# vovach777/llcomp

Measured on AMD Instinct MI355X. Metric: encode+decode MPix/s on 4K RGB8, bit-exact, higher is better.
Workload: dtype int32

## Files before the change

llcomp_amd/__init__.py:

```python
import ctypes as C
from collections import namedtuple

import numpy as np

from . import _lib
from ._lib import Info, Opts, OutputFormat

EXT = ".llcomp"
FORMAT_LEGACY, FORMAT_SLICED = 0, 1
(OK, BAD_MAGIC, BAD_EXPONENT, TRUNCATED, BAD_ARGS, OUT_OF_RANGE, OUTPUT_OVERFLOW, HIP_ERROR, NO_DEVICE, NOMEM, BUSY, DEVICE_FAILED) = range(12)
JOB_ENCODE, JOB_DECODE, JOB_DECODE_REGIONS, JOB_DECODE_RESIZED_REGIONS = 0, 1, 2, 3
DTYPE_U8, DTYPE_F32, DTYPE_F16, DTYPE_BF16 = 0, 1, 2, 3
LAYOUT_HWC, LAYOUT_CHW = 0, 1

RawImage = namedtuple("RawImage", "pixels width height channels")


class LlcompError(RuntimeError):
    def __init__(self, status, detail=None):
        self.status = int(status)
        msg = _lib.load().llcomp_mi_strerror(int(status)).decode()
        self.device_error = last_device_error() if self.status == DEVICE_FAILED else None
        super().__init__(msg if not detail else f"{msg} ({detail})")

# ... 626 lines not shown
    lens = (C.c_size_t * n)(*[len(b) for b in bands])
    out, m = _lib.u8p(), C.c_size_t()
    _check(L.llcomp_mi_merge_bands(ptrs, lens, n, C.byref(out), C.byref(m)))
    try:
        return C.string_at(out, m.value)
    finally:
        L.llcomp_mi_free(out)


def split_band(data, tile_row0, tile_row1):
    L = _lib.load()
    data = bytes(data)
    buf = (C.c_uint8 * max(1, len(data))).from_buffer_copy(data or b"\0")
    out, m = _lib.u8p(), C.c_size_t()
    _check(L.llcomp_mi_split_band(C.cast(buf, _lib.u8p), len(data), tile_row0, tile_row1, C.byref(out), C.byref(m)))
    try:
        return C.string_at(out, m.value)
    finally:
        L.llcomp_mi_free(out)


class Codec:

    def __init__(self, frames, w, h, c, tile_w=0, tile_h=0, planar=False, device=-1, small_model=False):
        self._L = _lib.load()
        self._h = C.c_void_p()
        _check(self._L.llcomp_mi_codec_create_ex(C.byref(self._h), device, frames, w, h, c, tile_w, tile_h, int(bool(planar)), 1 if small_model else 0))
        self.frames, self.w, self.h, self.c = frames, w, h, c
        self.n_slices = self._L.llcomp_mi_codec_slices(self._h)
        self.max_payload_bytes = self._L.llcomp_mi_codec_max_payload_bytes(self._h)
        self.workspace_bytes = self._L.llcomp_mi_codec_workspace_bytes(self._h)
        fam = self._L.llcomp_mi_codec_kernel_family(self._h)
        self.family = {"rows": bool(fam & 1), "lds_table": bool(fam & 2), "snapshot": bool(fam & 16), "bank_cache": bool(fam & 32),
                       "lane_shift": (fam >> 8) & 0xFF, "slices_per_wave": (fam >> 16) & 0xFF}

    def close(self):
        if self._h:
            self._L.llcomp_mi_codec_destroy(self._h)
            self._h = None

    __del__ = close

    def encode(self, d_px, d_payload, payload_cap, d_slice_len, d_total, d_status, stream=0):
        _check(self._L.llcomp_mi_codec_encode(self._h, d_px, d_payload, payload_cap, d_slice_len, d_total, d_status, stream))

    def decode(self, d_payload, payload_bytes, d_slice_len, d_px, d_status, stream=0):
        _check(self._L.llcomp_mi_codec_decode(self._h, d_payload, payload_bytes, d_slice_len, d_px, d_status, stream))

    def decode_region(self, d_payload, payload_bytes, d_slice_len, x, y, rw, rh, d_px, d_status, stream=0):
        _check(self._L.llcomp_mi_codec_decode_region(self._h, d_payload, payload_bytes, d_slice_len, x, y, rw, rh, d_px, d_status, stream))

    def encode_region(self, d_payload, payload_bytes, d_slice_len, x, y, rw, rh, d_rect, d_sub_payload, sub_payload_cap, d_sub_len, d_sub_total,
                      d_status, stream=0):
        _check(self._L.llcomp_mi_codec_encode_region(self._h, d_payload or None, payload_bytes, d_slice_len or None, x, y, rw, rh, d_rect,
                                                     d_sub_payload, sub_payload_cap, d_sub_len, d_sub_total, d_status, stream))

    def update_region(self, d_payload, payload_bytes, d_slice_len, x, y, rw, rh, d_rect, d_payload_out, payload_cap, d_slice_len_out, d_total,
                      d_status, stream=0):
        _check(self._L.llcomp_mi_codec_update_region(self._h, d_payload or None, payload_bytes, d_slice_len or None, x, y, rw, rh, d_rect,
                                                     d_payload_out, payload_cap, d_slice_len_out, d_total, d_status, stream))

    def region_family(self, x, y, rw, rh):
        fam = self._L.llcomp_mi_codec_region_family(self._h, x, y, rw, rh)
        if not fam:
            return None
        return {"rows": bool(fam & 1), "lds_table": bool(fam & 2), "snapshot": bool(fam & 16), "bank_cache": bool(fam & 32),
                "lane_shift": (fam >> 8) & 0xFF, "slices_per_wave": (fam >> 16) & 0xFF}
# ... 79 lines not shown
```

llcomp_amd/csrc/codec.hip:

```cpp
#include <hip/hip_runtime.h>

#include <algorithm>
#include <cstdlib>
#include <cstring>
#include <mutex>
#include <new>
#include <vector>

#include "../../include/llcomp_mi.h"
#include "codec_internal.hpp"
#include "container.hpp"
#include "geometry.hpp"
#include "kernels.hpp"
#include "resize.hpp"
#include "snapshot.hpp"
#include "tables.hpp"
#include "update.hpp"

using namespace llcomp_mi;

namespace llcomp_mi {

int status_from_bits(uint32_t bits) {
    if (bits & kStInternal) return LLCOMP_MI_HIP_ERROR;
// ... 741 lines not shown
    DeviceGuard guard(k->device);
    if (!guard.ok) return LLCOMP_MI_HIP_ERROR;
    if (what & LLCOMP_MI_PREPARE_ENCODE) {
        if (snapshot_mode(k->g)) {
            if (int rc = ensure_snapshot_arrays(k, k->g)) return rc;
        }
        if (!snapshot_mode(k->g) || snapshot_chunked(k->g))
            if (int rc = ensure_state_tables(k, k->need_states)) return rc;
    }
    if (what & LLCOMP_MI_PREPARE_DECODE)
        if (int rc = ensure_state_tables(k, k->need_states)) return rc;
    if (what & (LLCOMP_MI_PREPARE_REGION | LLCOMP_MI_PREPARE_REGIONS | LLCOMP_MI_PREPARE_RESIZED | LLCOMP_MI_PREPARE_UPDATE)) {
        if (int rc = ensure_region_arrays(k)) return rc;
        if (region_may_need_states(k))
            if (int rc = ensure_state_tables(k, true)) return rc;
    }
    if (what & LLCOMP_MI_PREPARE_REGIONS)
        if (int rc = ensure_regions_table(k)) return rc;
    if (what & LLCOMP_MI_PREPARE_UPDATE) {
        const uint64_t samples = uint64_t(k->g.frames) * k->g.w * k->g.h * k->g.c;
        if (int rc = ensure_update_arrays(k)) return rc;
        if (int rc = ensure_grown(k, k->d_box, k->box_cap, samples, samples)) return rc;
    }
    if (what & LLCOMP_MI_PREPARE_RESIZED) {
        const uint64_t samples = uint64_t(k->g.frames) * k->g.w * k->g.h * k->g.c;
        if (int rc = ensure_regions_ring(k)) return rc;
        if (int rc = ensure_grown(k, k->d_box, k->box_cap, samples, samples)) return rc;
        if (int rc = ensure_grown(k, k->d_mid, k->mid_cap, samples, samples)) return rc;
    }
    return LLCOMP_MI_OK;
}

uint32_t llcomp_mi_codec_slices(const llcomp_mi_codec* k) { return k ? k->g.n_slices : 0; }
uint32_t llcomp_mi_codec_kernel_family(const llcomp_mi_codec* k) { return k ? (k->g.flags & 0xFFu) | (k->g.lane_shift << 8) | (k->g.lpw << 16) : 0; }
uint64_t llcomp_mi_codec_workspace_bytes(const llcomp_mi_codec* k) { return k ? k->workspace_bytes : 0; }
uint64_t llcomp_mi_codec_allocated_bytes(const llcomp_mi_codec* k) { return k ? k->allocated_bytes : 0; }
uint64_t llcomp_mi_codec_max_payload_bytes(const llcomp_mi_codec* k) {
    return k ? uint64_t(k->g.n_slices) * k->g.slice_cap : 0;
}

int llcomp_mi_codec_model(llcomp_mi_codec* k, const void* d_px, void* d_sym, void* stream) {
    if (!k || !d_px || !d_sym) return LLCOMP_MI_BAD_ARGS;
    DeviceGuard guard(k->device);
    if (!guard.ok) return LLCOMP_MI_HIP_ERROR;
    HIP_TRY(launch_model_fwd(k->g, static_cast<const uint8_t*>(d_px), static_cast<uint32_t*>(d_sym),
                             static_cast<hipStream_t>(stream)));
    return LLCOMP_MI_OK;
}

int llcomp_mi_codec_encode(llcomp_mi_codec* k, const void* d_px, void* d_payload, uint64_t payload_cap, void* d_slice_len,
                           void* d_total, void* d_status, void* stream) {
    if (!k || !d_px || !d_payload || !d_slice_len || !d_total || !d_status) return LLCOMP_MI_BAD_ARGS;
    DeviceGuard guard(k->device);
    if (!guard.ok) return LLCOMP_MI_HIP_ERROR;
    hipStream_t s = static_cast<hipStream_t>(stream);
    DoneGuard done_guard{k, s};
    HIP_TRY(hipMemsetAsync(d_status, 0, 4, s));
    if (int rc = encode_streams(k, k->g, d_px, static_cast<uint32_t*>(d_slice_len), k->d_group_off, static_cast<uint32_t*>(d_status), s)) return rc;
    if (int rc = pack_streams(k, k->g, static_cast<const uint32_t*>(d_slice_len), k->d_group_off, static_cast<uint8_t*>(d_payload), payload_cap,
                              static_cast<uint64_t*>(d_total), static_cast<uint32_t*>(d_status), s))
        return rc;
    ++k->n_encode;
    return LLCOMP_MI_OK;
}

int llcomp_mi_codec_decode(llcomp_mi_codec* k, const void* d_payload, uint64_t payload_bytes, const void* d_slice_len,
                           void* d_px, void* d_status, void* stream) {
    if (!k || !d_payload || !d_slice_len || !d_px || !d_status) return LLCOMP_MI_BAD_ARGS;
    DeviceGuard guard(k->device);
    if (!guard.ok) return LLCOMP_MI_HIP_ERROR;
    hipStream_t s = static_cast<hipStream_t>(stream);
    const Geometry& g = k->g;
    DoneGuard done_guard{k, s};
    HIP_TRY(hipMemsetAsync(d_status, 0, 4, s));
    {
        Timed t(k, s, 7);
        if (int rc = next_state_generation(k, s, k->need_states)) return rc;
    }
    {
        Timed t(k, s, 4);
        HIP_TRY(launch_group_sums(g, static_cast<const uint32_t*>(d_slice_len), k->d_group_off, s));
        HIP_TRY(launch_scan_groups(g, k->d_group_off, k->d_total_tmp, s));
    }
    {
        Timed t(k, s, 4);
        HIP_TRY(launch_stage_streams(g, static_cast<const uint8_t*>(d_payload), payload_bytes,
                                     static_cast<const uint32_t*>(d_slice_len), k->d_group_off, k->d_scratch,
                                     static_cast<uint32_t*>(d_status), s));
    }
    {
        Timed t(k, s, 5);
        const bool cache = use_bank_cache(k, g);
        HIP_TRY(launch_decode_slices(g, k->d_scratch, static_cast<const uint32_t*>(d_slice_len), k->d_states, k->state_generation,
                                     static_cast<int16_t*>(k->d_lane_order), static_cast<uint32_t*>(d_status), k->d_counters, cache, s));
        if (cache) queue_feedback(k, s);
    }
    {
        Timed t(k, s, 6);
        if (model_is_fused(g)) {
            HIP_TRY(launch_model_rows_inv(g, static_cast<const int16_t*>(k->d_lane_order), static_cast<uint8_t*>(d_px), s));
        } else {
            HIP_TRY(launch_from_lane_order_i16(g, static_cast<const int16_t*>(k->d_lane_order),
                                               static_cast<int16_t*>(k->d_sym_or_rec), s));
            HIP_TRY(launch_model_inv(g, static_cast<const int16_t*>(k->d_sym_or_rec), static_cast<uint8_t*>(d_px), s));
        }
    }
    ++k->n_decode;
    return LLCOMP_MI_OK;
}

uint32_t llcomp_mi_codec_region_family(const llcomp_mi_codec* k, uint32_t x, uint32_t y, uint32_t rw, uint32_t rh) {
    RegionBox box;
    Geometry sub;
    if (!k || region_setup(k, x, y, rw, rh, box, sub)) return 0;
    return (sub.flags & 0xFFu) | (sub.lane_shift << 8) | (sub.lpw << 16);
}

int llcomp_mi_codec_decode_region(llcomp_mi_codec* k, const void* d_payload, uint64_t payload_bytes, const void* d_slice_len, uint32_t x,
                                  uint32_t y, uint32_t rw, uint32_t rh, void* d_px, void* d_status, void* stream) {
    if (!k || !d_payload || !d_slice_len || !d_px || !d_status) return LLCOMP_MI_BAD_ARGS;
    RegionBox box;
    Geometry sub;
    if (int rc = region_setup(k, x, y, rw, rh, box, sub)) return rc;
    DeviceGuard guard(k->device);
    if (!guard.ok) return LLCOMP_MI_HIP_ERROR;
    if (int rc = ensure_region_arrays(k)) return rc;
    hipStream_t s = static_cast<hipStream_t>(stream);
    const Geometry& g = k->g;
    DoneGuard done_guard{k, s};
    HIP_TRY(hipMemsetAsync(d_status, 0, 4, s));
    {
        Timed t(k, s, 7);
// ... 431 lines not shown
```

llcomp_amd/csrc/geometry.hpp:

```cpp
#pragma once
#include <algorithm>
#include <cstdint>
#include <cstdlib>

#if defined(__HIPCC__)
#define LLMI_HD __host__ __device__
#else
#define LLMI_HD
#endif

namespace llcomp_mi {

constexpr uint32_t kMaxChannels = 255;

struct Geometry {
    uint32_t frames, w, h, c;
    uint32_t tile_w, tile_h, planar;
    uint32_t ntx, nty;
    uint32_t slices_per_frame;
    uint32_t n_slices;
    uint32_t slice_cap;
    uint32_t nch;
    uint32_t lane_shift;
    uint32_t slice_samples;
    uint32_t lpw;
    uint32_t flags;
};
enum : uint32_t {
    kGeoRows = 1u,
    kGeoLdsTable = 2u,
    kGeoForceReplay = 4u,
    kGeoSmallModel = 8u,
    kGeoSnapshot = 16u,
    kGeoBankCache = 32u,
};
constexpr uint32_t kSnapMaxSamples = 4096;
constexpr uint32_t kSnapMaxChunks = 4;

struct Tuning {
    int lane_shift = -1;
    int lpw = 0;
    bool norows = false;
    bool noldstab = false;
    bool force_replay = false;
    bool nosnap = false;
    bool nocache = false;
    int overlap = 2;
    bool nofeedback = false;
};
inline Tuning tuning_from_env() {
    Tuning t;
    auto num = [](const char* name, long lo, long hi, int dflt) {
        const char* e = std::getenv(name);
        if (!e || !*e) return dflt;
        const long v = std::strtol(e, nullptr, 10);
        return (v >= lo && v <= hi) ? int(v) : dflt;
    };
    auto flag = [](const char* name) { const char* e = std::getenv(name); return e && e[0] == '1'; };
    t.lane_shift = num("LLCOMP_MI_LANE_SHIFT", 0, 6, -1);
    t.lpw = num("LLCOMP_MI_LPW", 1, 64, 0);
    t.norows = flag("LLCOMP_MI_NOROWS");
    t.noldstab = flag("LLCOMP_MI_NOLDSTAB");
    t.force_replay = flag("LLCOMP_MI_FORCE_REPLAY");
    t.nosnap = flag("LLCOMP_MI_NOSNAP");
    t.nocache = flag("LLCOMP_MI_NOCACHE");
    t.nofeedback = flag("LLCOMP_MI_NOFEEDBACK");
    t.overlap = num("LLCOMP_MI_OVERLAP", 0, 2, 2);
    return t;
}

LLMI_HD inline uint32_t snapshot_chunks(const Geometry& g) { return (g.slice_samples + kSnapMaxSamples - 1) / kSnapMaxSamples; }
LLMI_HD inline uint32_t snapshot_cap(const Geometry& g) {
    return g.slice_samples <= kSnapMaxSamples ? (g.slice_samples + 15u) & ~15u : snapshot_chunks(g) * kSnapMaxSamples;
}

constexpr int kBankCacheLog2 = 5;
inline int bank_cache_log2(const Geometry& g) { return (g.flags & kGeoBankCache) ? kBankCacheLog2 : 0; }

LLMI_HD inline uint32_t rows_px_dwords(uint64_t tile_base, uint32_t samples, uint32_t c, uint64_t batch_bytes) {
    if (tile_base + 4 > batch_bytes) return 0;
    const uint64_t k = (batch_bytes - 4 - tile_base) / c + 1;
    return k < samples ? uint32_t(k) : samples;
}
LLMI_HD inline uint32_t rows_px_tail(uint32_t c) { return 1 + (4 + c - 1) / c; }

LLMI_HD inline size_t lane_order_index(const Geometry& g, uint32_t id, uint32_t k) {
    const uint32_t gw = 1u << g.lane_shift;
    return ((size_t(id >> g.lane_shift) * g.slice_samples + k) << g.lane_shift) + (id & (gw - 1));
}

struct SliceRect {
    uint32_t frame, x0, y0, sw, sh, ch;
};

LLMI_HD inline SliceRect slice_rect(const Geometry& g, uint32_t id) {
    SliceRect r;
    r.frame = id / g.slices_per_frame;
    uint32_t s = id - r.frame * g.slices_per_frame;
    uint32_t tile = s;
    r.ch = 0;
    if (g.planar) {
        tile = s / g.c;
        r.ch = s - tile * g.c;
    }
    const uint32_t ty = tile / g.ntx, tx = tile - ty * g.ntx;
    r.x0 = tx * g.tile_w;
    r.y0 = ty * g.tile_h;
    r.sw = g.w - r.x0 < g.tile_w ? g.w - r.x0 : g.tile_w;
    r.sh = g.h - r.y0 < g.tile_h ? g.h - r.y0 : g.tile_h;
    return r;
}

inline uint32_t default_lane_shift(uint32_t n_slices) {
    constexpr uint32_t kMinWaves = 96;
    uint32_t s = 6;
    while (s > 0 && (n_slices >> s) < kMinWaves) --s;
    return s;
// ... 170 lines not shown
```

llcomp_amd/csrc/kernels.hpp:

```cpp
#pragma once
#include <hip/hip_runtime.h>

#include <cstdint>

#include "geometry.hpp"

namespace llcomp_mi {

enum : uint32_t { kStOverflow = 1u, kStBadExponent = 2u, kStTruncated = 4u, kStInternal = 8u  };

enum : uint32_t {
    kCtrDecCachedWaves = 0,
    kCtrDecBypassedWaves = 1,
    kCtrCacheLookups = 2,
    kCtrCacheMisses = 3,
    kCtrCacheWritebacks = 4,
    kCtrDecReplays = 5,
    kCtrEncCarryBacks = 6,
    kCtrGenerationWraps = 7,
    kCtrDecLaunchesCached = 8,
    kCtrDecLaunchesPlainByFeedback = 9,
    kCtrCount = 16,
};

hipError_t launch_model_fwd(const Geometry& g, const uint8_t* d_px, uint32_t* d_sym, hipStream_t stream);
hipError_t launch_model_inv(const Geometry& g, const int16_t* d_rec, uint8_t* d_px, hipStream_t stream);

uint32_t lane_groups(const Geometry& g);
uint32_t slice_capacity_samples(const Geometry& g);
hipError_t launch_to_lane_order_u32(const Geometry& g, const uint32_t* d_img, uint32_t* d_lanes, hipStream_t stream);
hipError_t launch_from_lane_order_i16(const Geometry& g, const int16_t* d_lanes, int16_t* d_img, hipStream_t stream);

bool model_is_fused(const Geometry& g);
bool rows_encoder_reads_pixels(const Geometry& g);
hipError_t launch_model_rows_fwd(const Geometry& g, const uint8_t* d_px, uint16_t* d_lanes, hipStream_t stream);
hipError_t launch_model_rows_inv(const Geometry& g, const int16_t* d_lanes, uint8_t* d_px, hipStream_t stream);

bool rows_mode(const Geometry& g);
bool slices_need_state_tables(const Geometry& g);

hipError_t launch_encode_slices(const Geometry& g, const void* d_sym, uint64_t* d_states, uint32_t generation, uint8_t* d_scratch,
                                uint32_t* d_slice_len, uint64_t* d_group_off, uint32_t* d_status, unsigned long long* d_counters,
                                hipStream_t stream);
uint64_t state_generation_tag(uint32_t generation);
hipError_t launch_encode_segment(const Geometry& g, const void* d_res, uint64_t* d_banks, uint8_t* d_scratch, uint32_t* d_slice_len,
                                 uint32_t* d_status, unsigned long long* d_counters, uint32_t seg_first, uint32_t* d_seg_state,
                                 hipStream_t stream);
bool encoder_writes_group_sums(const Geometry& g);
hipError_t launch_group_sums(const Geometry& g, const uint32_t* d_slice_len, uint64_t* d_group_off, hipStream_t stream);
hipError_t launch_scan_groups(const Geometry& g, uint64_t* d_group_off, uint64_t* d_total, hipStream_t stream);
hipError_t launch_frame_bytes(const Geometry& g, const uint32_t* d_slice_len, uint64_t* d_frame_bytes, hipStream_t stream);
hipError_t launch_pack_payload(const Geometry& g, const uint8_t* d_units, const uint32_t* d_slice_len,
                               const uint64_t* d_group_off, uint8_t* d_payload, uint64_t payload_cap,
                               uint32_t* d_status, hipStream_t stream);
hipError_t launch_stage_streams(const Geometry& g, const uint8_t* d_payload, uint64_t payload_bytes,
                                const uint32_t* d_slice_len, const uint64_t* d_group_off, uint8_t* d_units,
                                uint32_t* d_status, hipStream_t stream);
hipError_t launch_copy_segments(const uint8_t* d_src, uint8_t* d_dst, const uint64_t* d_src_off, const uint64_t* d_dst_off,
                                const uint64_t* d_len, uint32_t n_seg, uint64_t max_len, hipStream_t stream);
hipError_t launch_range_sums(const uint32_t* d_vals, const uint64_t* d_start, const uint64_t* d_count, uint64_t* d_out, uint32_t n,
                             uint32_t cap, hipStream_t stream);
hipError_t launch_decode_slices(const Geometry& g, const uint8_t* d_units, const uint32_t* d_slice_len,
                                uint64_t* d_states, uint32_t generation, int16_t* d_rec, uint32_t* d_status, unsigned long long* d_counters,
                                bool bank_cache, hipStream_t stream);

hipError_t launch_region_index(const Geometry& full, const Geometry& sub, const RegionBox& box, const uint32_t* d_slice_len,
                               const uint64_t* d_group_off, uint32_t* d_sub_len, uint64_t* d_sub_off, hipStream_t stream);
hipError_t launch_stage_region_streams(const Geometry& sub, const uint8_t* d_payload, uint64_t payload_bytes, const uint32_t* d_sub_len,
                                       const uint64_t* d_sub_off, uint8_t* d_units, uint32_t* d_status, hipStream_t stream);
struct Crop {
    uint32_t x0, y0, rw, rh;
};
hipError_t launch_model_inv_crop(const Geometry& sub, const int16_t* d_rec, uint8_t* d_px, const Crop& cr, hipStream_t stream);
hipError_t launch_model_rows_inv_crop(const Geometry& sub, const int16_t* d_lanes, uint8_t* d_px, const Crop& cr, hipStream_t stream);

hipError_t launch_regions_index(const Geometry& full, const Geometry& sub, const RegionsFrame* d_tab, const uint32_t* d_slice_len,
                                const uint64_t* d_group_off, uint32_t* d_sub_len, uint64_t* d_sub_off, hipStream_t stream);
hipError_t launch_model_inv_crops(const Geometry& sub, const int16_t* d_rec, uint8_t* d_px, const RegionsFrame* d_tab, uint32_t rw,
                                  uint32_t rh, hipStream_t stream);
hipError_t launch_model_rows_inv_crops(const Geometry& sub, const int16_t* d_lanes, uint8_t* d_px, const RegionsFrame* d_tab, uint32_t rw,
                                       uint32_t rh, hipStream_t stream);

}
```

llcomp_amd/csrc/model_kernels.hip:

```cpp
#include <algorithm>

#include "device_common.hpp"
#include "kernels.hpp"

namespace llcomp_mi {

namespace {

constexpr int kMW = 256;
constexpr int kMH = 32;

template <int C>
__device__ __forceinline__ void rct_forward(const uint8_t* p, int16_t (&o)[C]) {
    if constexpr (C >= 3) {
        const int g = p[1], cb = int(p[2]) - g, cr = int(p[0]) - g;
        o[0] = int16_t(cr);
        o[1] = int16_t(g + (cb + cr) / 4);
        o[2] = int16_t(cb);
        if constexpr (C == 4) o[3] = p[3];
    } else {
#pragma unroll
        for (int k = 0; k < C; ++k) o[k] = p[k];
    }
}
// ... 813 lines not shown
        uint8_t bytes[4 * C];
#pragma unroll
        for (int i = 0; i < 4; ++i) {
            const int16_t* s = &tile[4 * q4 + i][col0 + tt * C];
            if constexpr (C >= 3) {
                int r = s[0], gg = s[1], bb = s[2];
                gg -= (r + bb) / 4;
                r += gg;
                bb += gg;
                bytes[i * C + 0] = uint8_t(min(max(r, 0), 255));
                bytes[i * C + 1] = uint8_t(min(max(gg, 0), 255));
                bytes[i * C + 2] = uint8_t(min(max(bb, 0), 255));
                if constexpr (C == 4) bytes[i * C + 3] = uint8_t(s[3]);
            } else {
#pragma unroll
                for (int c = 0; c < C; ++c) bytes[i * C + c] = uint8_t(s[c]);
            }
        }
        uint8_t* o = px + tiles[tt].base + size_t(kb) * C;
        const uint32_t npx = sw - kb < 4 ? sw - kb : 4;
        if (npx == 4) {
            uint32_t w[C];
#pragma unroll
            for (int c = 0; c < C; ++c)
                w[c] = uint32_t(bytes[4 * c]) | (uint32_t(bytes[4 * c + 1]) << 8) | (uint32_t(bytes[4 * c + 2]) << 16) |
                       (uint32_t(bytes[4 * c + 3]) << 24);
            __builtin_memcpy(o, w, 4 * C);
        } else {
            for (uint32_t i = 0; i < npx * C; ++i) o[i] = bytes[i];
        }
    }
}

struct RowTileCrop {
    long long base;
    uint32_t klo, khi;
};
template <int C>
__device__ __forceinline__ void load_row_tiles_crop(const Geometry& g, uint32_t first_tile, uint32_t ntiles, const Crop& cr,
                                                    RowTileCrop* tiles) {
    if (threadIdx.x < ntiles) {
        const uint32_t tile = first_tile + threadIdx.x;
        const uint32_t per_frame = g.ntx * g.nty;
        const uint32_t frame = tile / per_frame, rem = tile - frame * per_frame;
        const uint32_t y = rem / g.ntx, tx = rem - y * g.ntx;
        const uint32_t x0 = tx * g.tile_w;
        const uint32_t sw = g.w - x0 < g.tile_w ? g.w - x0 : g.tile_w;
        const uint32_t klo = cr.x0 > x0 ? cr.x0 - x0 : 0u;
        uint32_t khi = cr.x0 + cr.rw > x0 ? min(sw, cr.x0 + cr.rw - x0) : 0u;
        if (y < cr.y0 || y >= cr.y0 + cr.rh || khi <= klo) khi = 0;
        tiles[threadIdx.x].base = ((long long)(size_t(frame) * cr.rh + (y - cr.y0)) * cr.rw + (long long)x0 - (long long)cr.x0) * C;
        tiles[threadIdx.x].klo = klo;
        tiles[threadIdx.x].khi = khi;
    }
}
template <int C>
__global__ __launch_bounds__(256) void k_model_rows_inv_crop(const Geometry g, const int16_t* __restrict__ lanes,
                                                             uint8_t* __restrict__ px, const Crop cr) {
    constexpr int K = 64, TPG = 64 / C + 2;
    __shared__ __attribute__((aligned(4))) int16_t tile[K][64 + C + 1 + ((C + 1) & 1)];
    __shared__ RowTileCrop tiles[TPG];
    const uint32_t chunks = (g.tile_w + K - 1) / K;
    uint32_t group, chunk;
    if (!xcd_chunk_group((g.n_slices + (1u << g.lane_shift) - 1) >> g.lane_shift, chunks, group, chunk)) return;
    const uint32_t k0 = chunk * K;
    const uint32_t gw = 1u << g.lane_shift;
// ... 237 lines not shown
    }
    const uint32_t nbx = (g.w + kMW - 1) / kMW;
    const uint32_t spt = (g.tile_h + kMH - 1) / kMH;
    const uint64_t blocks = uint64_t(nbx) * spt * g.nty * g.frames;
    if (blocks == 0 || blocks > 0x7FFFFFFFull) return hipErrorInvalidValue;
    LLMI_DISPATCH_C(g.c, (k_model_fwd<C><<<dim3(uint32_t(blocks)), dim3(kMW), 0, stream>>>(g, d_px, d_sym)));
    return hipGetLastError();
}

uint32_t lane_groups(const Geometry& g) { return (g.n_slices + (1u << g.lane_shift) - 1) >> g.lane_shift; }
uint32_t slice_capacity_samples(const Geometry& g) { return g.slice_samples; }

hipError_t launch_to_lane_order_u32(const Geometry& g, const uint32_t* d_img, uint32_t* d_lanes, hipStream_t stream) {
    const uint32_t max_n = slice_capacity_samples(g);
    const uint64_t blocks = uint64_t(lane_groups(g)) * ((max_n + 63) / 64);
    if (blocks == 0 || blocks > 0x7FFFFFFFull) return hipErrorInvalidValue;
    k_to_lane_order<uint32_t><<<dim3(uint32_t(blocks)), dim3(256), 0, stream>>>(g, max_n, d_img, d_lanes);
    return hipGetLastError();
}

hipError_t launch_from_lane_order_i16(const Geometry& g, const int16_t* d_lanes, int16_t* d_img, hipStream_t stream) {
    const uint32_t max_n = slice_capacity_samples(g);
    const uint64_t blocks = uint64_t(lane_groups(g)) * ((max_n + 63) / 64);
    if (blocks == 0 || blocks > 0x7FFFFFFFull) return hipErrorInvalidValue;
    k_from_lane_order<int16_t><<<dim3(uint32_t(blocks)), dim3(256), 0, stream>>>(g, max_n, d_lanes, d_img);
    return hipGetLastError();
}

bool model_is_fused(const Geometry& g) { return g.planar && rows_mode(g) && g.c <= 4; }
bool rows_encoder_reads_pixels(const Geometry& g) {
    return model_is_fused(g) && (uint64_t(63 / g.c + 2) * g.tile_w * g.c + 4 < (1ull << 31));
}

hipError_t launch_model_rows_fwd(const Geometry& g, const uint8_t* d_px, uint16_t* d_lanes, hipStream_t stream) {
    const uint64_t blocks = xcd_grid(lane_groups(g), (g.tile_w + 63) / 64);
    if (blocks == 0 || blocks > 0x7FFFFFFFull) return hipErrorInvalidValue;
    LLMI_DISPATCH_C(g.c, (k_model_rows_fwd<C><<<dim3(uint32_t(blocks)), dim3(256), 0, stream>>>(g, d_px, d_lanes)));
    return hipGetLastError();
}

hipError_t launch_model_rows_inv(const Geometry& g, const int16_t* d_lanes, uint8_t* d_px, hipStream_t stream) {
    const uint64_t blocks = xcd_chunk_grid(lane_groups(g), (g.tile_w + 63) / 64);
    if (blocks == 0 || blocks > 0x7FFFFFFFull) return hipErrorInvalidValue;
    LLMI_DISPATCH_C(g.c, (k_model_rows_inv<C><<<dim3(uint32_t(blocks)), dim3(256), 0, stream>>>(g, d_lanes, d_px)));
    return hipGetLastError();
}

hipError_t launch_model_inv(const Geometry& g, const int16_t* d_rec, uint8_t* d_px, hipStream_t stream) {
    const size_t npix = size_t(g.frames) * g.h * g.w;
    if (g.c > 4) {
        k_model_inv_any<<<dim3(uint32_t((npix + 255) / 256)), dim3(256), 0, stream>>>(g, d_rec, d_px, npix);
        return hipGetLastError();
    }
    const uint32_t blocks = uint32_t(std::min<size_t>((npix + 255) / 256, 256 * 16));
    LLMI_DISPATCH_C(g.c, (k_model_inv<C><<<dim3(blocks), dim3(256), 0, stream>>>(g, d_rec, d_px, npix)));
    return hipGetLastError();
}

hipError_t launch_group_sums(const Geometry& g, const uint32_t* d_slice_len, uint64_t* d_group_off, hipStream_t stream) {
    k_group_sums<<<dim3((g.n_slices + kSumThreads - 1) / kSumThreads), dim3(kSumThreads), 0, stream>>>(d_slice_len, g.n_slices, g.lane_shift, d_group_off);
    return hipGetLastError();
}

hipError_t launch_frame_bytes(const Geometry& g, const uint32_t* d_slice_len, uint64_t* d_frame_bytes, hipStream_t stream) {
    k_frame_bytes<<<dim3(g.frames), dim3(256), 0, stream>>>(d_slice_len, g.slices_per_frame, d_frame_bytes);
    return hipGetLastError();
// ... 109 lines not shown
```

llcomp_amd/csrc/slice_kernels.hip:

```cpp
#include <algorithm>

#include "device_common.hpp"
#include "kernels.hpp"

#ifndef LLMI_ASM_ENC
#define LLMI_ASM_ENC 1
#endif
#if LLMI_ASM_ENC
#include "enc_rows_asm.hpp"
#endif
#ifndef LLMI_ASM_DEC
#define LLMI_ASM_DEC 1
#endif
#if LLMI_ASM_DEC
#include "dec_rows_asm.hpp"
#endif

namespace llcomp_mi {

namespace {

#ifdef LLMI_CLOCK_PROBE
constexpr uint32_t kProbeSlots = 1u << 15;
__device__ unsigned long long g_probe[2][kProbeSlots][2];
// ... 859 lines not shown
                                           uint32_t& v) {
    const uint32_t s_low = d.low, s_range = d.range, s_b0 = bank.w[0], s_b1 = bank.w[1], s_b2 = bank.w[2], s_b3 = bank.w[3];
    const unsigned long long s_win = d.win;
    bool ok;
#if LLMI_ASM_DEC
    if constexpr (INLDS) {
        uint32_t left;
        dec_rows_sample_asm(d.low, d.range, d.win, bank.w[0], bank.w[1], bank.w[2], bank.w[3], lds_address(bank.lds), hot, v, left);
        ok = left != 0;
    } else
#endif
    {
        ok = hot ? dec_residual<true, false, INLDS>(d, bank, tab, v) : dec_residual<false, false, INLDS>(d, bank, tab, v);
        hot = 2 * __popcll(__ballot(v != 0)) >= __popcll(__ballot(true));
    }
    const bool ran_dry = (INLDS && LLMI_ASM_DEC != 0) ? false : d.win == 0;
    if (__builtin_expect(!ok || ran_dry || replay_always, 0)) {
        ++d.replays;
        d.low = s_low; d.range = s_range; d.win = s_win;
        bank.w[0] = s_b0; bank.w[1] = s_b1;
        if constexpr (INLDS) {
            bank.w[2] = s_b2; bank.w[3] = s_b3;
            reinterpret_cast<uint32_t*>(bank.lds)[0] = s_b0;
            reinterpret_cast<uint32_t*>(bank.lds)[64] = s_b1;
            reinterpret_cast<uint32_t*>(bank.lds)[128] = s_b2;
            reinterpret_cast<uint32_t*>(bank.lds)[192] = s_b3;
        }
        ok = dec_residual<false, true, INLDS>(d, bank, tab, v);
    }
    return ok;
}

constexpr uint32_t bank_cache_lds_bytes(int log2_entries) { return log2_entries ? (64u * 9u) << log2_entries : 0u; }
template <int NCH, bool ROWS, bool LDSTAB = false, int CACHE = 0>
__global__ __launch_bounds__(64) void k_decode_slices(const Geometry g, const uint32_t lpw_and_flags,
                                                      const uint8_t* __restrict__ units,
                                                      const uint32_t* __restrict__ slice_len,
                                                      uint64_t* __restrict__ states, int16_t* __restrict__ rec,
                                                      uint32_t* status, const uint64_t gpat,
                                                      unsigned long long* __restrict__ counters) {
    __shared__ entry_t tab[128];
    __shared__ uint32_t rowbank[ROWS ? kWideBankWords : 1];
    __shared__ int8_t quant_lut[ROWS ? 1 : 512];
    if constexpr (!ROWS) {
        for (uint32_t i = threadIdx.x; i < 256; i += blockDim.x) {
            quant_lut[i] = int8_t(quant11(int(i) - 128));
            quant_lut[256 + i] = int8_t(quant5(int(i) - 128));
        }
    }
    static_assert(CACHE == 0 || (!ROWS && !LDSTAB && NCH != 0), "the bank cache belongs to the 2-D kernels with tables in HBM");
    static_assert(CACHE == 0 || ((kContexts - 1) >> CACHE) < 0xFF, "bank cache: a context's tag would alias the empty marker");
    __shared__ uint32_t wave_sums[CACHE != 0 ? 2 : 1];
    clear_lds_states<LDSTAB>();
    if constexpr (CACHE != 0) {
        uint32_t* tg = reinterpret_cast<uint32_t*>(dyn_lds + (512u << CACHE));
        for (uint32_t i = threadIdx.x; i < (16u << CACHE); i += blockDim.x) tg[i] = 0xFFFFFFFFu;
        if (threadIdx.x < 2) wave_sums[threadIdx.x] = 0;
    }
    load_table(tab);
    const uint32_t lpw = lpw_and_flags & 0xFF;
    const bool replay_always = (lpw_and_flags >> 8) & 1;
    const bool small_model = (g.flags & kGeoSmallModel) != 0;
    const uint32_t id = blockIdx.x * lpw + threadIdx.x;
    if (threadIdx.x >= lpw || id >= g.n_slices) return;
    const SliceRect r = slice_rect(g, id);
    RangeDec d;
    const uint32_t len = min(slice_len[id], g.slice_cap - 16);
    const uint32_t grp = __builtin_amdgcn_readfirstlane(id >> g.lane_shift);
    const uint32_t lane_in_group = id & ((1u << g.lane_shift) - 1);
    dec_open(d, reinterpret_cast<const uint32_t*>(units) + ((size_t(grp) * (g.slice_cap >> 2)) << g.lane_shift), lane_in_group,
             g.lane_shift, len);

    int16_t* p0 = rec + lane_order_index(g, id, 0);
    const ptrdiff_t GW = ptrdiff_t(1) << g.lane_shift;
    int16_t* const gbase = rec + ((size_t(grp) * g.slice_samples) << g.lane_shift);
    uint32_t hot = 0;
    LLMI_PROBE_START();

    if constexpr (ROWS) {
        for (uint32_t k = 0; k < 12; ++k) rowbank[k * 64 + threadIdx.x] = lds_address(tab) * 0x00010001u;
        int l[NCH], L[NCH];
#pragma unroll
        for (int k = 0; k < NCH; ++k) l[k] = L[k] = 128;
        int held_val = 0;
        uint32_t held_ofs = lane_in_group * 2, next_ofs = held_ofs, step_ofs = 2u << g.lane_shift;
        uint32_t large = small_model ? 0u : ~0u, first = ~0u;
        asm volatile("" : "+v"(large), "+v"(first), "+v"(step_ofs));
        uint8_t* const bank0 = reinterpret_cast<uint8_t*>(rowbank) + threadIdx.x * 4;
        bool bad = false;
        auto pixel = [&]() {
#pragma unroll
            for (int k = 0; k < NCH; ++k) {
                if (window_low(d)) dec_append(d);
                asm volatile("global_store_short %0, %1, %2" : : "v"(held_ofs), "v"(held_val), "s"(gbase) : "memory");
                const int lv = l[k];
                const int dq = (L[k] - lv) & int(large);
                int sg = dq >> 31;
                asm volatile("" : "+v"(sg));
                const uint32_t aq = uint32_t((dq ^ sg) - sg);
                uint32_t o1 = ((aq + 0x7FFFFFFFu) >> 21) & 0x400u, o2 = ((aq + 0x7FFFFFFCu) >> 21) & 0x400u;
                asm volatile("" : "+v"(o1), "+v"(o2));
                uint32_t* bp = reinterpret_cast<uint32_t*>(bank0 + (o1 + o2));
                Bank bank{{bp[0], bp[64], bp[128], bp[192]}, reinterpret_cast<uint8_t*>(bp)};
                uint32_t v = 0;
                if (!dec_sample<true>(d, bank, tab, hot, replay_always, v)) bad = true;
                v = (v ^ uint32_t(sg)) - uint32_t(sg);
                const int val = int(int16_t(uint32_t(lv) + v));
                held_val = val;
                held_ofs = next_ofs;
                next_ofs += step_ofs;
                L[k] = lv ^ ((lv ^ val) & int(first));
                l[k] = val;
            }
            first = 0;
        };
        const uint32_t sw0 = __builtin_amdgcn_readfirstlane(r.sw);
        const uint32_t n_bulk = __builtin_amdgcn_ballot_w64(r.sw != sw0) == 0 ? sw0 : 0;
        uint32_t x = 0;
        for (; x < n_bulk; ++x) pixel();
        for (; x < r.sw; ++x) pixel();
        if (bad) atomicOr(status, kStBadExponent);
        asm volatile("global_store_short %0, %1, %2" : : "v"(held_ofs), "v"(held_val), "s"(gbase) : "memory");
        publish_count(counters, kCtrDecReplays, d.replays);
    } else {
        uint64_t* banks;
        uint32_t bsh;
        if constexpr (LDSTAB) {
            banks = reinterpret_cast<uint64_t*>(dyn_lds);
            bsh = 0;
        } else {
            banks = states + ((size_t(id >> g.lane_shift) * kContexts) << g.lane_shift) + (id & ((1u << g.lane_shift) - 1));
            bsh = g.lane_shift;
        }
        if constexpr (NCH == 0) {
            const uint32_t nch = g.nch;
            const ptrdiff_t px_step = ptrdiff_t(nch) * GW, up = ptrdiff_t(r.sw) * px_step;
            for (uint32_t y = 0; y < r.sh; ++y) {
                for (uint32_t x = 0; x < r.sw; ++x) {
                    for (uint32_t k = 0; k < nch; ++k) {
                        int16_t* q = p0 + ptrdiff_t(y) * up + ptrdiff_t(x) * px_step + ptrdiff_t(k) * GW;
                        if (window_low(d)) dec_append(d);
                        const Hood n = apply_borders(x > 0 ? q[-px_step] : 0, x > 1 ? q[-2 * px_step] : 0, y > 0 ? q[-up] : 0,
                                                     (y > 0 && x > 0) ? q[-up - px_step] : 0, (y > 0 && x + 1 < r.sw) ? q[-up + px_step] : 0,
                                                     y > 1 ? q[-2 * up] : 0, x, y, r.sw);
                        int ctx = context_hash(n, small_model);
                        const bool neg = ctx < 0;
                        if (neg) ctx = -ctx;
                        const uint64_t b64 = bank_fresh<LDSTAB>(banks[size_t(ctx) << bsh], gpat);
                        Bank bank{{uint32_t(b64), uint32_t(b64 >> 32)}, nullptr};
                        uint32_t v;
                        if (!dec_sample<false>(d, bank, tab, hot, replay_always, v)) {
                            atomicOr(status, kStBadExponent);
                            return;
                        }
                                banks[size_t(ctx) << bsh] = bank_tagged<LDSTAB>(uint64_t(bank.w[0]) | (uint64_t(bank.w[1]) << 32), gpat);
// ... 220 lines not shown
    const uint32_t lpw = g.lpw;
    const uint32_t blocks = (g.n_slices + lpw - 1) / lpw;
    uint64_t* const d_group_sum = encoder_writes_group_sums(g) ? d_group_off : nullptr;
    if (rows_encoder_reads_pixels(g)) {
        k_encode_slices<1, true, uint8_t><<<dim3(blocks), dim3(64), LLMI_ASM_ENC ? kRowsEncLdsBytes : 0, stream>>>(
            g, lpw, static_cast<const uint8_t*>(d_sym), d_states, d_scratch, d_slice_len, d_group_sum, d_status, gpat, d_counters);
        return hipGetLastError();
    }
    if (model_is_fused(g)) {
        k_encode_slices<1, true, uint16_t><<<dim3(blocks), dim3(64), LLMI_ASM_ENC ? kRowsEncLdsBytes : 0, stream>>>(
            g, lpw, static_cast<const uint16_t*>(d_sym), d_states, d_scratch, d_slice_len, d_group_sum, d_status, gpat, d_counters);
        return hipGetLastError();
    }
    if (g.flags & kGeoSnapshot) {
        k_encode_slices<0, false, uint32_t, false, true><<<dim3(blocks), dim3(64), LLMI_ASM_ENC ? kRowsEncLdsBytes : 0, stream>>>(
            g, lpw, static_cast<const uint32_t*>(d_sym), d_states, d_scratch, d_slice_len, d_group_sum, d_status, 0, d_counters);
        return hipGetLastError();
    }
    const bool lds = states_in_lds(g);
    LLMI_DISPATCH_SLICE(g.nch, rows_mode(g), lds, {
        auto kernel = k_encode_slices<C, R, uint32_t, T>;
        if (T) {
            const hipError_t e = allow_big_lds(kernel);
            if (e != hipSuccess) return e;
        }
        kernel<<<dim3(blocks), dim3(64), T ? kLdsTableBytes : (R && LLMI_ASM_ENC ? kRowsEncLdsBytes : 0), stream>>>(
            g, lpw, static_cast<const uint32_t*>(d_sym), d_states, d_scratch, d_slice_len, d_group_sum, d_status, gpat, d_counters, 0u, nullptr);
    });
    return hipGetLastError();
}

hipError_t launch_decode_slices(const Geometry& g, const uint8_t* d_units, const uint32_t* d_slice_len,
                                uint64_t* d_states, uint32_t generation, int16_t* d_rec, uint32_t* d_status, unsigned long long* d_counters,
                                bool bank_cache, hipStream_t stream) {
    const uint64_t gpat = slices_need_state_tables(g) ? state_generation_tag(generation) : 0;
    const uint32_t lpw = g.lpw;
    const uint32_t blocks = (g.n_slices + lpw - 1) / lpw;
    const uint32_t arg = lpw | ((g.flags & kGeoForceReplay) ? 0x100u : 0u);
    const bool lds = states_in_lds(g);
    if (bank_cache_log2(g) == kBankCacheLog2 && bank_cache) {
#define LLMI_DECODE_CACHED(NCHV)                                                                                          \
    k_decode_slices<NCHV, false, false, kBankCacheLog2><<<dim3(blocks), dim3(64), bank_cache_lds_bytes(kBankCacheLog2), stream>>>( \
        g, arg, d_units, d_slice_len, d_states, d_rec, d_status, gpat, d_counters)
        switch (g.nch) {
            case 1: LLMI_DECODE_CACHED(1); break;
            case 2: LLMI_DECODE_CACHED(2); break;
            case 3: LLMI_DECODE_CACHED(3); break;
            case 4: LLMI_DECODE_CACHED(4); break;
            default: return hipErrorInvalidValue;
        }
#undef LLMI_DECODE_CACHED
        return hipGetLastError();
    }
    LLMI_DISPATCH_SLICE(g.nch, rows_mode(g), lds, {
        auto kernel = k_decode_slices<C, R, T>;
        if (T) {
            const hipError_t e = allow_big_lds(kernel);
            if (e != hipSuccess) return e;
        }
        kernel<<<dim3(blocks), dim3(64), T ? kLdsTableBytes : 0, stream>>>(g, arg, d_units, d_slice_len, d_states,
                                                                          d_rec, d_status, gpat, d_counters);
    });
    return hipGetLastError();
}

}
```

Baseline: 28890.

## Fuse inverse color model and pixel write into the rows slice decoder

The planar rows decoder now stages decoded samples in LDS and, every eight pixels, applies the inverse RGB transform and writes packed 8-byte pixel words straight to the output image. This removes the separate inverse-model pass over the lane-order buffer. Tiles whose channels span two waves still write int16 samples, and a small straddle kernel converts those afterwards. The price is extra LDS staging and wave barriers inside the serial decode loop, plus partial-store handling at tile edges. An env flag can turn the fused path off.

```diff
diff --git a/llcomp_amd/__init__.py b/llcomp_amd/__init__.py
--- a/llcomp_amd/__init__.py
+++ b/llcomp_amd/__init__.py
@@ -682,7 +682,8 @@
         self.workspace_bytes = self._L.llcomp_mi_codec_workspace_bytes(self._h)
         fam = self._L.llcomp_mi_codec_kernel_family(self._h)
         self.family = {"rows": bool(fam & 1), "lds_table": bool(fam & 2), "snapshot": bool(fam & 16), "bank_cache": bool(fam & 32),
-                       "lane_shift": (fam >> 8) & 0xFF, "slices_per_wave": (fam >> 16) & 0xFF}
+                       "lane_shift": (fam >> 8) & 0xFF, "slices_per_wave": (fam >> 16) & 0xFF,
+                       "px_decoder": bool(fam & (1 << 24))}
 
     def close(self):
         if self._h:
diff --git a/llcomp_amd/csrc/codec.hip b/llcomp_amd/csrc/codec.hip
--- a/llcomp_amd/csrc/codec.hip
+++ b/llcomp_amd/csrc/codec.hip
@@ -797,7 +797,11 @@
 }
 
 uint32_t llcomp_mi_codec_slices(const llcomp_mi_codec* k) { return k ? k->g.n_slices : 0; }
-uint32_t llcomp_mi_codec_kernel_family(const llcomp_mi_codec* k) { return k ? (k->g.flags & 0xFFu) | (k->g.lane_shift << 8) | (k->g.lpw << 16) : 0; }
+uint32_t llcomp_mi_codec_kernel_family(const llcomp_mi_codec* k) {
+    if (!k) return 0;
+    const uint32_t px_decoder = rows_decoder_writes_pixels(k->g) && !k->tune.nofuseddec ? 1u << 24 : 0u;
+    return (k->g.flags & 0xFFu) | (k->g.lane_shift << 8) | (k->g.lpw << 16) | px_decoder;
+}
 uint64_t llcomp_mi_codec_workspace_bytes(const llcomp_mi_codec* k) { return k ? k->workspace_bytes : 0; }
 uint64_t llcomp_mi_codec_allocated_bytes(const llcomp_mi_codec* k) { return k ? k->allocated_bytes : 0; }
 uint64_t llcomp_mi_codec_max_payload_bytes(const llcomp_mi_codec* k) {
@@ -853,16 +857,20 @@
                                      static_cast<const uint32_t*>(d_slice_len), k->d_group_off, k->d_scratch,
                                      static_cast<uint32_t*>(d_status), s));
     }
+    const bool px_decoder = rows_decoder_writes_pixels(g) && !k->tune.nofuseddec;
     {
         Timed t(k, s, 5);
         const bool cache = use_bank_cache(k, g);
         HIP_TRY(launch_decode_slices(g, k->d_scratch, static_cast<const uint32_t*>(d_slice_len), k->d_states, k->state_generation,
-                                     static_cast<int16_t*>(k->d_lane_order), static_cast<uint32_t*>(d_status), k->d_counters, cache, s));
+                                     static_cast<int16_t*>(k->d_lane_order), static_cast<uint32_t*>(d_status), k->d_counters, cache, s,
+                                     px_decoder ? static_cast<uint8_t*>(d_px) : nullptr));
         if (cache) queue_feedback(k, s);
     }
     {
         Timed t(k, s, 6);
-        if (model_is_fused(g)) {
+        if (px_decoder) {
+            HIP_TRY(launch_model_rows_inv_straddle(g, static_cast<const int16_t*>(k->d_lane_order), static_cast<uint8_t*>(d_px), s));
+        } else if (model_is_fused(g)) {
             HIP_TRY(launch_model_rows_inv(g, static_cast<const int16_t*>(k->d_lane_order), static_cast<uint8_t*>(d_px), s));
         } else {
             HIP_TRY(launch_from_lane_order_i16(g, static_cast<const int16_t*>(k->d_lane_order),
diff --git a/llcomp_amd/csrc/geometry.hpp b/llcomp_amd/csrc/geometry.hpp
--- a/llcomp_amd/csrc/geometry.hpp
+++ b/llcomp_amd/csrc/geometry.hpp
@@ -47,6 +47,7 @@
     bool nocache = false;
     int overlap = 2;
     bool nofeedback = false;
+    bool nofuseddec = false;
 };
 inline Tuning tuning_from_env() {
     Tuning t;
@@ -65,6 +66,7 @@
     t.nosnap = flag("LLCOMP_MI_NOSNAP");
     t.nocache = flag("LLCOMP_MI_NOCACHE");
     t.nofeedback = flag("LLCOMP_MI_NOFEEDBACK");
+    t.nofuseddec = flag("LLCOMP_MI_NOFUSEDDEC");
     t.overlap = num("LLCOMP_MI_OVERLAP", 0, 2, 2);
     return t;
 }
@@ -83,6 +85,20 @@
     return k < samples ? uint32_t(k) : samples;
 }
 LLMI_HD inline uint32_t rows_px_tail(uint32_t c) { return 1 + (4 + c - 1) / c; }
+
+constexpr uint32_t kRowsFlush = 8;
+LLMI_HD inline bool rows_tile_in_wave(const Geometry& g, uint32_t id) {
+    const uint32_t first = id - id % g.lpw, end = g.n_slices - first < g.lpw ? g.n_slices : first + g.lpw;
+    const uint32_t t0 = id - id % g.c;
+    return t0 >= first && t0 + g.c <= end;
+}
+LLMI_HD inline uint32_t rows_flush_bytes(uint32_t n, uint32_t c, uint32_t plane) {
+    const uint32_t nb = n * c, lo = 8 * plane;
+    return nb > lo ? (nb - lo < 8 ? nb - lo : 8u) : 0u;
+}
+LLMI_HD constexpr uint32_t rows_flush_pixels(uint32_t c) { return c == 3 ? 4u : 8u / c; }
+LLMI_HD inline uint32_t rows_flush_first_pixel(uint32_t c, uint32_t plane) { return c == 3 ? 2 * plane : 8 * plane / c; }
+LLMI_HD inline size_t rows_straddle_index(const Geometry& g, uint32_t id, uint32_t k) { return size_t(id) * g.slice_samples + k; }
 
 LLMI_HD inline size_t lane_order_index(const Geometry& g, uint32_t id, uint32_t k) {
     const uint32_t gw = 1u << g.lane_shift;
diff --git a/llcomp_amd/csrc/kernels.hpp b/llcomp_amd/csrc/kernels.hpp
--- a/llcomp_amd/csrc/kernels.hpp
+++ b/llcomp_amd/csrc/kernels.hpp
@@ -35,6 +35,9 @@
 bool rows_encoder_reads_pixels(const Geometry& g);
 hipError_t launch_model_rows_fwd(const Geometry& g, const uint8_t* d_px, uint16_t* d_lanes, hipStream_t stream);
 hipError_t launch_model_rows_inv(const Geometry& g, const int16_t* d_lanes, uint8_t* d_px, hipStream_t stream);
+bool rows_decoder_writes_pixels(const Geometry& g);
+bool rows_straddlers(const Geometry& g);
+hipError_t launch_model_rows_inv_straddle(const Geometry& g, const int16_t* d_rec, uint8_t* d_px, hipStream_t stream);
 
 bool rows_mode(const Geometry& g);
 bool slices_need_state_tables(const Geometry& g);
@@ -62,7 +65,7 @@
                              uint32_t cap, hipStream_t stream);
 hipError_t launch_decode_slices(const Geometry& g, const uint8_t* d_units, const uint32_t* d_slice_len,
                                 uint64_t* d_states, uint32_t generation, int16_t* d_rec, uint32_t* d_status, unsigned long long* d_counters,
-                                bool bank_cache, hipStream_t stream);
+                                bool bank_cache, hipStream_t stream, uint8_t* d_px = nullptr);
 
 hipError_t launch_region_index(const Geometry& full, const Geometry& sub, const RegionBox& box, const uint32_t* d_slice_len,
                                const uint64_t* d_group_off, uint32_t* d_sub_len, uint64_t* d_sub_off, hipStream_t stream);
diff --git a/llcomp_amd/csrc/model_kernels.hip b/llcomp_amd/csrc/model_kernels.hip
--- a/llcomp_amd/csrc/model_kernels.hip
+++ b/llcomp_amd/csrc/model_kernels.hip
@@ -869,6 +869,36 @@
     }
 }
 
+constexpr uint32_t kStraddleThreads = 256;
+template <int C>
+__global__ __launch_bounds__(kStraddleThreads) void k_model_rows_inv_straddle(const Geometry g, const int16_t* __restrict__ rec, uint8_t* __restrict__ px) {
+    const uint32_t chunks = (g.tile_w + kStraddleThreads - 1) / kStraddleThreads;
+    const uint32_t m = blockIdx.x / chunks + 1, chunk = blockIdx.x - (m - 1) * chunks;
+    const uint32_t b = m * g.lpw;
+    const uint32_t id0 = b - b % C;
+    if (b == id0 || (b - g.lpw > id0)) return;
+    const SliceRect r = slice_rect(g, id0);
+    const uint32_t k = chunk * kStraddleThreads + threadIdx.x;
+    if (k >= r.sw) return;
+    int s[C];
+#pragma unroll
+    for (int c = 0; c < C; ++c) s[c] = rec[rows_straddle_index(g, id0 + c, k)];
+    uint8_t* o = px + ((size_t(r.frame) * g.h + r.y0) * g.w + r.x0 + k) * C;
+    if constexpr (C >= 3) {
+        int rr = s[0], gg = s[1], bb = s[2];
+        gg -= (rr + bb) / 4;
+        rr += gg;
+        bb += gg;
+        o[0] = uint8_t(min(max(rr, 0), 255));
+        o[1] = uint8_t(min(max(gg, 0), 255));
+        o[2] = uint8_t(min(max(bb, 0), 255));
+        if constexpr (C == 4) o[3] = uint8_t(s[3]);
+    } else {
+#pragma unroll
+        for (int c = 0; c < C; ++c) o[c] = uint8_t(s[c]);
+    }
+}
+
 struct RowTileCrop {
     long long base;
     uint32_t klo, khi;
@@ -1172,6 +1202,18 @@
     return model_is_fused(g) && (uint64_t(63 / g.c + 2) * g.tile_w * g.c + 4 < (1ull << 31));
 }
 
+bool rows_decoder_writes_pixels(const Geometry& g) { return rows_encoder_reads_pixels(g); }
+bool rows_straddlers(const Geometry& g) { return g.lpw % g.c != 0 && g.n_slices > g.lpw; }
+
+hipError_t launch_model_rows_inv_straddle(const Geometry& g, const int16_t* d_rec, uint8_t* d_px, hipStream_t stream) {
+    if (!rows_decoder_writes_pixels(g)) return hipErrorInvalidValue;
+    if (!rows_straddlers(g)) return hipSuccess;
+    const uint64_t blocks = uint64_t((g.n_slices - 1) / g.lpw) * ((g.tile_w + kStraddleThreads - 1) / kStraddleThreads);
+    if (blocks == 0 || blocks > 0x7FFFFFFFull) return hipErrorInvalidValue;
+    LLMI_DISPATCH_C(g.c, (k_model_rows_inv_straddle<C><<<dim3(uint32_t(blocks)), dim3(kStraddleThreads), 0, stream>>>(g, d_rec, d_px)));
+    return hipGetLastError();
+}
+
 hipError_t launch_model_rows_fwd(const Geometry& g, const uint8_t* d_px, uint16_t* d_lanes, hipStream_t stream) {
     const uint64_t blocks = xcd_grid(lane_groups(g), (g.tile_w + 63) / 64);
     if (blocks == 0 || blocks > 0x7FFFFFFFull) return hipErrorInvalidValue;
diff --git a/llcomp_amd/csrc/slice_kernels.hip b/llcomp_amd/csrc/slice_kernels.hip
--- a/llcomp_amd/csrc/slice_kernels.hip
+++ b/llcomp_amd/csrc/slice_kernels.hip
@@ -915,15 +915,66 @@
 }
 
 constexpr uint32_t bank_cache_lds_bytes(int log2_entries) { return log2_entries ? (64u * 9u) << log2_entries : 0u; }
-template <int NCH, bool ROWS, bool LDSTAB = false, int CACHE = 0>
+using lds_i16_ptr = __attribute__((address_space(3))) int16_t*;
+__device__ __forceinline__ void rows_inv_rgb(int& r, int& gg, int& bb) {
+    gg -= (r + bb) / 4;
+    r += gg;
+    bb += gg;
+    r = min(max(r, 0), 255);
+    gg = min(max(gg, 0), 255);
+    bb = min(max(bb, 0), 255);
+}
+__device__ __forceinline__ uint32_t pack4(uint32_t b0, uint32_t b1, uint32_t b2, uint32_t b3) { return b0 | (b1 << 8) | (b2 << 16) | (b3 << 24); }
+template <int C>
+__device__ __forceinline__ void rows_flush_words(lds_i16_ptr q, uint32_t sh, uint32_t& w0, uint32_t& w1) {
+    if constexpr (C == 3) {
+        uint32_t b[12];
+#pragma unroll
+        for (int j = 0; j < 4; ++j) {
+            lds_i16_ptr s = q + j * 64;
+            int r = s[0], gg = s[1], bb = s[2];
+            rows_inv_rgb(r, gg, bb);
+            b[3 * j] = uint32_t(r);
+            b[3 * j + 1] = uint32_t(gg);
+            b[3 * j + 2] = uint32_t(bb);
+        }
+        const uint32_t W0 = pack4(b[0], b[1], b[2], b[3]), W1 = pack4(b[4], b[5], b[6], b[7]), W2 = pack4(b[8], b[9], b[10], b[11]);
+        w0 = uint32_t((W0 | ((unsigned long long)W1 << 32)) >> sh);
+        w1 = uint32_t((W1 | ((unsigned long long)W2 << 32)) >> sh);
+    } else if constexpr (C == 4) {
+        uint32_t w[2];
+#pragma unroll
+        for (int j = 0; j < 2; ++j) {
+            lds_i16_ptr s = q + j * 64;
+            int r = s[0], gg = s[1], bb = s[2];
+            const uint32_t a = uint8_t(s[3]);
+            rows_inv_rgb(r, gg, bb);
+            w[j] = pack4(uint32_t(r), uint32_t(gg), uint32_t(bb), a);
+        }
+        w0 = w[0];
+        w1 = w[1];
+    } else {
+        uint32_t b[8];
+#pragma unroll
+        for (int j = 0; j < 8 / C; ++j)
+#pragma unroll
+            for (int c = 0; c < C; ++c) b[j * C + c] = uint8_t(q[j * 64 + c]);
+        w0 = pack4(b[0], b[1], b[2], b[3]);
+        w1 = pack4(b[4], b[5], b[6], b[7]);
+    }
+}
+
+template <int NCH, bool ROWS, bool LDSTAB = false, int CACHE = 0, int PXC = 0>
 __global__ __launch_bounds__(64) void k_decode_slices(const Geometry g, const uint32_t lpw_and_flags,
                                                       const uint8_t* __restrict__ units,
                                                       const uint32_t* __restrict__ slice_len,
                                                       uint64_t* __restrict__ states, int16_t* __restrict__ rec,
                                                       uint32_t* status, const uint64_t gpat,
-                                                      unsigned long long* __restrict__ counters) {
+                                                      unsigned long long* __restrict__ counters, uint8_t* __restrict__ px) {
+    static_assert(PXC == 0 || (ROWS && NCH == 1 && PXC <= 4), "the pixel form belongs to the planar 1-row kernels");
     __shared__ entry_t tab[128];
     __shared__ uint32_t rowbank[ROWS ? kWideBankWords : 1];
+    __shared__ int16_t stage[PXC != 0 ? kRowsFlush * 64 : 1];
     __shared__ int8_t quant_lut[ROWS ? 1 : 512];
     if constexpr (!ROWS) {
         for (uint32_t i = threadIdx.x; i < 256; i += blockDim.x) {
@@ -965,17 +1016,71 @@
         int l[NCH], L[NCH];
 #pragma unroll
         for (int k = 0; k < NCH; ++k) l[k] = L[k] = 128;
-        int held_val = 0;
-        uint32_t held_ofs = lane_in_group * 2, next_ofs = held_ofs, step_ofs = 2u << g.lane_shift;
+        [[maybe_unused]] int held_val = 0;
+        [[maybe_unused]] uint32_t held_ofs = lane_in_group * 2, next_ofs = held_ofs, step_ofs = 2u << g.lane_shift;
         uint32_t large = small_model ? 0u : ~0u, first = ~0u;
-        asm volatile("" : "+v"(large), "+v"(first), "+v"(step_ofs));
+        if constexpr (PXC == 0) asm volatile("" : "+v"(large), "+v"(first), "+v"(step_ofs));
+        else asm volatile("" : "+v"(large), "+v"(first));
         uint8_t* const bank0 = reinterpret_cast<uint8_t*>(rowbank) + threadIdx.x * 4;
+        [[maybe_unused]] lds_i16_ptr st_w = nullptr, st_r = nullptr;
+        [[maybe_unused]] bool whole = false;
+        [[maybe_unused]] uint32_t out_ofs = 0, px_sh = 0;
+        [[maybe_unused]] uint8_t* gpx = nullptr;
+        [[maybe_unused]] char* grec = nullptr;
+        if constexpr (PXC != 0) {
+            const uint32_t wfirst = blockIdx.x * lpw;
+            whole = rows_tile_in_wave(g, id);
+            const unsigned long long tbase = ((unsigned long long)(r.frame) * g.h + r.y0) * g.w * PXC + (unsigned long long)(r.x0) * PXC;
+            const unsigned long long wbase = (unsigned long long)uint32_t(__builtin_amdgcn_readfirstlane(uint32_t(tbase))) |
+                                             ((unsigned long long)uint32_t(__builtin_amdgcn_readfirstlane(uint32_t(tbase >> 32))) << 32);
+            gpx = px + wbase;
+            grec = reinterpret_cast<char*>(rec + rows_straddle_index(g, wfirst, 0));
+            const uint32_t q0 = rows_flush_first_pixel(PXC, r.ch);
+            lds_i16_ptr const st = (lds_i16_ptr)stage;
+            st_w = st + threadIdx.x;
+            st_r = whole ? st + (threadIdx.x - r.ch) + q0 * 64 : st + threadIdx.x;
+            px_sh = 8 * (8 * r.ch - PXC * q0);
+            asm volatile("" : "+v"(px_sh));
+            out_ofs = whole ? uint32_t(tbase - wbase) + 8 * r.ch : uint32_t(rows_straddle_index(g, id, 0) - rows_straddle_index(g, wfirst, 0)) * 2;
+        }
+        [[maybe_unused]] auto flush = [&](uint32_t n, auto full) {
+            constexpr bool FULL = decltype(full)::value;
+            __builtin_amdgcn_wave_barrier();
+            if (whole) {
+                uint32_t w0, w1;
+                rows_flush_words<(PXC != 0 ? PXC : 1)>(st_r, px_sh, w0, w1);
+                uint8_t* o = gpx + out_ofs;
+                const uint32_t nb = FULL ? 8u : rows_flush_bytes(n, PXC, PXC == 3 ? px_sh >> 4 : r.ch);
+                if (nb == 8) {
+                    const uint2 w = make_uint2(w0, w1);
+                    __builtin_memcpy(o, &w, 8);
+                } else {
+                    unsigned long long ww = w0 | ((unsigned long long)w1 << 32);
+                    for (uint32_t i = 0; i < nb; ++i, ww >>= 8) o[i] = uint8_t(ww);
+                }
+                out_ofs += 8u * PXC;
+            } else {
+                char* o = grec + out_ofs;
+                if (FULL) {
+                    uint32_t w[4];
+#pragma unroll
+                    for (int j = 0; j < 4; ++j) w[j] = uint32_t(uint16_t(st_r[2 * j * 64])) | (uint32_t(uint16_t(st_r[(2 * j + 1) * 64])) << 16);
+                    const uint4 w4 = make_uint4(w[0], w[1], w[2], w[3]);
+                    __builtin_memcpy(o, &w4, 16);
+                } else {
+                    for (uint32_t i = 0; i < n; ++i) reinterpret_cast<int16_t*>(o)[i] = st_r[i * 64];
+                }
+                out_ofs += 16u;
+            }
+            if constexpr (FULL) st_w -= kRowsFlush * 64;
+        };
         bool bad = false;
-        auto pixel = [&]() {
+        auto pixel = [&](auto&& behind_topup) {
 #pragma unroll
             for (int k = 0; k < NCH; ++k) {
                 if (window_low(d)) dec_append(d);
-                asm volatile("global_store_short %0, %1, %2" : : "v"(held_ofs), "v"(held_val), "s"(gbase) : "memory");
+                if constexpr (PXC == 0) asm volatile("global_store_short %0, %1, %2" : : "v"(held_ofs), "v"(held_val), "s"(gbase) : "memory");
+                else behind_topup();
                 const int lv = l[k];
                 const int dq = (L[k] - lv) & int(large);
                 int sg = dq >> 31;
@@ -989,21 +1094,37 @@
                 if (!dec_sample<true>(d, bank, tab, hot, replay_always, v)) bad = true;
                 v = (v ^ uint32_t(sg)) - uint32_t(sg);
                 const int val = int(int16_t(uint32_t(lv) + v));
-                held_val = val;
-                held_ofs = next_ofs;
-                next_ofs += step_ofs;
+                if constexpr (PXC == 0) {
+                    held_val = val;
+                    held_ofs = next_ofs;
+                    next_ofs += step_ofs;
+                } else {
+                    *st_w = int16_t(val);
+                    st_w += 64;
+                }
                 L[k] = lv ^ ((lv ^ val) & int(first));
                 l[k] = val;
             }
             first = 0;
         };
+        auto nothing = [] {};
         const uint32_t sw0 = __builtin_amdgcn_readfirstlane(r.sw);
         const uint32_t n_bulk = __builtin_amdgcn_ballot_w64(r.sw != sw0) == 0 ? sw0 : 0;
         uint32_t x = 0;
-        for (; x < n_bulk; ++x) pixel();
-        for (; x < r.sw; ++x) pixel();
+        if constexpr (PXC == 0) {
+            for (; x < n_bulk; ++x) pixel(nothing);
+            for (; x < r.sw; ++x) pixel(nothing);
+        } else {
+            for (const uint32_t n_blk = n_bulk & ~(kRowsFlush - 1); x < n_blk; x += kRowsFlush) {
+                pixel([&] { if (x != 0) flush(kRowsFlush, std::true_type{}); });
+#pragma unroll 1
+                for (uint32_t j = 1; j < kRowsFlush; ++j) pixel(nothing);
+            }
+            for (; x < r.sw; ++x) pixel([&] { if ((x & (kRowsFlush - 1)) == 0 && x != 0) flush(kRowsFlush, std::true_type{}); });
+            flush(((r.sw - 1) & (kRowsFlush - 1)) + 1, std::false_type{});
+        }
         if (bad) atomicOr(status, kStBadExponent);
-        asm volatile("global_store_short %0, %1, %2" : : "v"(held_ofs), "v"(held_val), "s"(gbase) : "memory");
+        if constexpr (PXC == 0) asm volatile("global_store_short %0, %1, %2" : : "v"(held_ofs), "v"(held_val), "s"(gbase) : "memory");
         publish_count(counters, kCtrDecReplays, d.replays);
     } else {
         uint64_t* banks;
@@ -1290,16 +1411,30 @@
 
 hipError_t launch_decode_slices(const Geometry& g, const uint8_t* d_units, const uint32_t* d_slice_len,
                                 uint64_t* d_states, uint32_t generation, int16_t* d_rec, uint32_t* d_status, unsigned long long* d_counters,
-                                bool bank_cache, hipStream_t stream) {
+                                bool bank_cache, hipStream_t stream, uint8_t* d_px) {
     const uint64_t gpat = slices_need_state_tables(g) ? state_generation_tag(generation) : 0;
     const uint32_t lpw = g.lpw;
     const uint32_t blocks = (g.n_slices + lpw - 1) / lpw;
     const uint32_t arg = lpw | ((g.flags & kGeoForceReplay) ? 0x100u : 0u);
+    if (d_px) {
+        if (!rows_decoder_writes_pixels(g)) return hipErrorInvalidValue;
+#define LLMI_DECODE_PX(CV)                                                                                              \
+    k_decode_slices<1, true, false, 0, CV><<<dim3(blocks), dim3(64), 0, stream>>>(g, arg, d_units, d_slice_len, d_states, d_rec, d_status, \
+                                                                                   gpat, d_counters, d_px)
+        switch (g.c) {
+            case 1: LLMI_DECODE_PX(1); break;
+            case 2: LLMI_DECODE_PX(2); break;
+            case 3: LLMI_DECODE_PX(3); break;
+            default: LLMI_DECODE_PX(4); break;
+        }
+#undef LLMI_DECODE_PX
+        return hipGetLastError();
+    }
     const bool lds = states_in_lds(g);
     if (bank_cache_log2(g) == kBankCacheLog2 && bank_cache) {
 #define LLMI_DECODE_CACHED(NCHV)                                                                                          \
     k_decode_slices<NCHV, false, false, kBankCacheLog2><<<dim3(blocks), dim3(64), bank_cache_lds_bytes(kBankCacheLog2), stream>>>( \
-        g, arg, d_units, d_slice_len, d_states, d_rec, d_status, gpat, d_counters)
+        g, arg, d_units, d_slice_len, d_states, d_rec, d_status, gpat, d_counters, nullptr)
         switch (g.nch) {
             case 1: LLMI_DECODE_CACHED(1); break;
             case 2: LLMI_DECODE_CACHED(2); break;
@@ -1317,7 +1452,7 @@
             if (e != hipSuccess) return e;
         }
         kernel<<<dim3(blocks), dim3(64), T ? kLdsTableBytes : 0, stream>>>(g, arg, d_units, d_slice_len, d_states,
-                                                                          d_rec, d_status, gpat, d_counters);
+                                                                          d_rec, d_status, gpat, d_counters, nullptr);
     });
     return hipGetLastError();
 }
```

Result: faster. 29870 (median of 6 runs) (+3.4%).
